# NVlabs/GLAMR

Measured on AMD Instinct MI355X. Metric: sequences/sec (300-frame, 1-person) end-to-end global_recon, higher is better.
Workload: dtype f32 (optimiser, init_data) / fp16x2-split MFMA with f32 accumulation (priors, LBS: every f32 operand as hi + lo fp16 planes, hi*hi + hi*lo + lo*hi)

## Files before the change

glamr_amd/csrc/nets.hip:

```cpp
#include "common.hpp"
#include "nn_kernels.hpp"
#include "nn_free.hpp"
#include "block_rt.hpp"
#include "rotmath.hpp"
#include <vector>
#include <cmath>
#include <cstring>
#include <map>
#include <mutex>

using namespace glamr;
using namespace glamr::nn;

namespace {

constexpr int D = 256, FF = 512, NZ = 128, WIN = 50, PAST = 10, CUR = 30, XLD = 96;

struct Lin { float* W = nullptr; float* b = nullptr; int N = 0, K = 0; unsigned short* Ws = nullptr;
             double rowabs = 0, babs = 0, wabs = 0; };
struct LN { float* g = nullptr; float* b = nullptr; double bound = 0; };
struct EncLayer { Lin qkv, o, f1, f2; LN n1, n2; };
struct DecLayer { Lin sa_qkv, sa_o, ca_q, ca_kv, ca_o, f1, f2; LN n1, n2, n3; };

struct HostT {
// ... 299 lines not shown
  __syncthreads();
  rt.scan(xy, n, 2, false);
  rt.scan(xy + 1, n, 2, false);
  for (int t = threadIdx.x; t < max_len; t += blockDim.x) {
    float tr[3] = {0.f, 0.f, 0.f}, aa[3] = {0.f, 0.f, 0.f};
    if (t < n) {
      const float base[4] = {0.5f, 0.5f, 0.5f, 0.5f};
      float hq[4], R[9], lq[4], q1[4], q[4];
      rm::heading_quat(theta[t], hq);
      rm::rot6d_to_rotmat(L + t * 11 + 3, R);
      rm::rotmat_to_quat(R, lq);
      rm::quat_mul(hq, lq, q1);
      rm::quat_mul(q1, base, q);
      rm::quat_to_aa(q, aa);
      tr[0] = xy[t * 2]; tr[1] = xy[t * 2 + 1]; tr[2] = L[t * 11 + 2];
    }
    for (int c = 0; c < 3; ++c) { trans[((size_t)b * max_len + t) * 3 + c] = tr[c]; orient[((size_t)b * max_len + t) * 3 + c] = aa[c]; }
  }
}

struct Ws {
  float *pose, *x, *h0, *h1, *qkv, *att, *tmp, *ff, *ctxkv, *qbuf, *pz, *z, *zproj, *dq, *y;
  float *tx, *tg, *th, *tq, *tmean, *trow, *traw, *tscr;
  float *gx, *q2, *qpz;
  float *te, *tcat, *e6, *tqz, *tloc;
  unsigned char* mask; int* lens; int* lens2;
  size_t total; int Tpad;
};
Ws ws_layout(int B, int max_len, char* base) {
  Ws w{};
  int nwin = (max_len - PAST + CUR - 1) / CUR;
  if (nwin < 1) nwin = 1;
  w.Tpad = std::max(max_len, (nwin - 1) * CUR + WIN);
  size_t off = 0;
  auto take = [&](size_t nfloats) { float* p = reinterpret_cast<float*>(base + off); off = align_up(off + (nfloats + 32 * 1024) * sizeof(float), 256); return p; };
  const size_t MW = (size_t)B * WIN, MT = (size_t)B * max_len;
  w.pose = take((size_t)B * w.Tpad * XLD);
  w.x = take(MW * XLD); w.h0 = take(MW * D); w.h1 = take(MW * D); w.qkv = take(MW * 3 * D); w.att = take(MW * D); w.tmp = take(MW * D);
  w.ff = take(MW * FF); w.ctxkv = take(MW * 2 * D); w.qbuf = take(MW * D); w.pz = take((size_t)B * 2 * D); w.z = take((size_t)B * NZ);
  w.zproj = take((size_t)B * FF); w.dq = take(MW * D); w.y = take(MW * 128);
  w.tx = take(MT * XLD); w.tg = take(MT * 1024); w.th = take(MT * D); w.tq = take(MT * D); w.tmean = take((size_t)B * D); w.trow = take((size_t)B * FF);
  w.traw = take(MT * 64); w.tscr = take(MT * 3);
  w.gx = take(MW * XLD); w.q2 = take((size_t)B * 2 * D); w.qpz = take((size_t)B * 2 * D);
  w.te = take(MT * D); w.tcat = take(MT * FF); w.e6 = take(MT * 32); w.tqz = take((size_t)B * D); w.tloc = take(MT * 11);
  w.mask = reinterpret_cast<unsigned char*>(take((MW + 3) / 4 + 64));
  w.lens = reinterpret_cast<int*>(take((size_t)B + 64));
  w.lens2 = reinterpret_cast<int*>(take((size_t)B + 64));
  w.total = off;
  return w;
}

#define RC(expr) do { int _rc = (expr); if (_rc) return _rc; } while (0)

thread_local int tl_fp32 = 0;
thread_local int tl_free = 0;
inline size_t cp(int col) { return tl_free ? (size_t)col * 32 : (size_t)col; }
inline bool free_wanted(int flags) {
  const char* e = std::getenv("GLAMR_NETS_FREE");
  return e ? std::atoi(e) != 0 : (flags & GLAMR_NETS_COSCHEDULE) != 0;
}

__global__ __launch_bounds__(64) void attention_f32_kernel(const float* Q, int ldq, const float* K, const float* V, int ldk, const unsigned char* key_mask,
                                                           float* O, int ldo, int Lq, int Lk, int q_shared) {
  __shared__ float sK[64][33], sV[64][33];
  __shared__ unsigned char sM[64];
  const int b = blockIdx.x, h = blockIdx.y, lane = threadIdx.x;
  for (int idx = lane; idx < 64 * 32; idx += 64) {
    const int j = idx >> 5, d = idx & 31;
    sK[j][d] = j < Lk ? K[(size_t)(b * Lk + j) * ldk + h * 32 + d] : 0.f;
    sV[j][d] = j < Lk ? V[(size_t)(b * Lk + j) * ldk + h * 32 + d] : 0.f;
  }
  sM[lane] = (lane < Lk) ? (key_mask ? key_mask[(size_t)b * Lk + lane] : 0) : 1;
  __syncthreads();
  if (lane >= Lq) return;
  float q[32], sc[64], o[32];
  for (int d = 0; d < 32; ++d) { q[d] = Q[(size_t)((q_shared ? 0 : b * Lq) + lane) * ldq + h * 32 + d]; o[d] = 0.f; }
  float mx = -3.0e38f;
  for (int j = 0; j < Lk; ++j) {
    float s = 0.f;
    for (int d = 0; d < 32; ++d) s = fmaf(q[d], sK[j][d], s);
    sc[j] = s * 0.17677669529663687f;
    if (!sM[j]) mx = fmaxf(mx, sc[j]);
  }
  float sum = 0.f;
  for (int j = 0; j < Lk; ++j) { const float e = sM[j] ? 0.f : expf(sc[j] - mx); sc[j] = e; sum += e; }
  const float inv = sum > 0.f ? 1.0f / sum : 0.f;
  for (int j = 0; j < Lk; ++j) { const float p = sc[j] * inv; for (int d = 0; d < 32; ++d) o[d] = fmaf(p, sV[j][d], o[d]); }
  for (int d = 0; d < 32; ++d) O[(size_t)(b * Lq + lane) * ldo + h * 32 + d] = o[d];
}

template <class... A>
void launch_attention(dim3 grid, dim3 block, size_t lds, hipStream_t st, const float* Q, int ldq, const float* K, const float* V, int ldk,
                      const unsigned char* mask, float* O, int ldo, int Lq, int Lk, int q_shared) {
  if (tl_fp32) hipLaunchKernelGGL(attention_f32_kernel, grid, dim3(64), 0, st, Q, ldq, K, V, ldk, mask, O, ldo, Lq, Lk, q_shared);
  else if (tl_free) hipLaunchKernelGGL(attention_free_kernel, dim3(grid.x * 8), dim3(64), 0, st, Q, ldq, K, V, ldk, mask, O, ldo, Lq, Lk, q_shared);
  else hipLaunchKernelGGL(attention_mfma_kernel, grid, block, lds, st, Q, ldq, K, V, ldk, mask, O, ldo, Lq, Lk, q_shared);
}

int ln(hipStream_t st, const float* X, const float* R, const LN& n, float* Y, int rows) {
  if (tl_free) { hipLaunchKernelGGL(ln_free_kernel, dim3((rows + 31) / 32), dim3(64), 0, st, X, R, n.g, n.b, Y, rows); return GLAMR_OK; }
  hipLaunchKernelGGL(add_layernorm_kernel, dim3((rows + 3) / 4), dim3(256), 0, st, X, R, n.g, n.b, Y, rows, D);
  return GLAMR_OK;
}
static const int FUSE_MIN_ROWS = [] { const char* e = std::getenv("GLAMR_NETS_FUSE_MIN_ROWS"); return e ? std::atoi(e) : 2048; }();
inline bool fuse_attention(int M) {
  static const bool no_fuse = std::getenv("GLAMR_NETS_NO_FUSE_ATTN") != nullptr || std::getenv("GLAMR_NETS_NO_FUSE") != nullptr;
  return !no_fuse && !tl_fp32 && !tl_free && M >= FUSE_MIN_ROWS;
}
int proj_ln(hipStream_t st, const Lin& L, const LN& n, const float* X, const float* R, float* Y, float* tmp, int M);
int mlp2(hipStream_t st, const Lin& L1, const Lin& L2, const LN* n, const float* X, int ldx, const float* R, float* Y, float* hidden, float* tmp, int M,
         int act2, int xl = -1);

inline bool small_rows_split(const Lin& L, int M, int ldx, int ldy, int ldr, int ldrb, bool bwd) {
  static const bool keep_fp32 = std::getenv("GLAMR_GEMM_SMALL_FP32") != nullptr || std::getenv("GLAMR_GEMM_FP32_MFMA") != nullptr;
  static const bool fwd_too = std::getenv("GLAMR_GEMM_SMALL_SPLIT_FWD") != nullptr;
  if (!bwd && !fwd_too) return false;
  return !keep_fp32 && !tl_fp32 && L.Ws && M > 0 && M < 2048 && L.K % 32 == 0 && ldx % 4 == 0 && ldy % 4 == 0 && ldr % 4 == 0 && ldrb % 4 == 0;
}

int lin(hipStream_t st, const Lin& L, const float* X, int ldx, float* Y, int ldy, int M, int act = ACT_NONE, const float* R = nullptr, int ldr = 0,
        const float* rowbias = nullptr, int rpg = 1, int ldrb = 0, int xl = -1, int yl = -1, bool bwd = false) {
  if (tl_free && L.Ws && M > 0) {
    if (L.K % 32 != 0 || ldx % 4 != 0 || ldy % 4 != 0) return fail(GLAMR_E_INVALID, "gemm: K=%d must be a multiple of 32, ldx=%d / ldy=%d of 4", L.K, ldx, ldy);
    GemmArgs a{X, L.W, L.b, rowbias, R, Y, M, L.N, L.K, ldx, ldy, ldr, rpg, ldrb, act};
    a.Ws = L.Ws;
    a.ws_plane = (size_t)((L.N + 63) / 64 * 64) * L.K;
    a.x_frag = xl != 0;
    a.y_frag = yl != 0;
    return launch_gemm_free(st, a);
  }
  if (small_rows_split(L, M, ldx, ldy, R ? ldr : 4, rowbias ? ldrb : 4, bwd)) {
    GemmArgs a{X, L.W, L.b, rowbias, R, Y, M, L.N, L.K, ldx, ldy, ldr, rpg, ldrb, act};
    a.Ws = L.Ws;
    a.ws_plane = (size_t)((L.N + 63) / 64 * 64) * L.K;
    return launch_gemm_free(st, a);
  }
  return launch_gemm(st, X, ldx, L.W, L.b, Y, ldy, M, L.N, L.K, act, R, ldr, rowbias, rpg, ldrb, L.Ws);
}

int proj_ln(hipStream_t st, const Lin& L, const LN& n, const float* X, const float* R, float* Y, float* tmp, int M) {
  static const bool no_fuse = std::getenv("GLAMR_NETS_NO_FUSE") != nullptr;
  if (!no_fuse && !tl_free && M >= FUSE_MIN_ROWS && L.N == D && L.K == D && L.Ws)
    return launch_rows(st, X, D, M, D, nullptr, 0, nullptr, nullptr, 1, 0, L.Ws, (size_t)D * L.K, L.K, L.b, ACT_NONE, R, D, n.g, n.b, Y, D);
  static const bool res_in_ln = std::getenv("GLAMR_NETS_RES_IN_LN") != nullptr;
  if (tl_free && !res_in_ln) {
    RC(lin(st, L, X, D, tmp, D, M, ACT_NONE, R, D));
    return ln(st, tmp, nullptr, n, Y, M);
  }
  RC(lin(st, L, X, D, tmp, D, M));
  return ln(st, tmp, R, n, Y, M);
}
int mlp2(hipStream_t st, const Lin& L1, const Lin& L2, const LN* n, const float* X, int ldx, const float* R, float* Y, float* hidden, float* tmp, int M,
         int act2, int xl) {
  static const bool no_fuse = std::getenv("GLAMR_NETS_NO_FUSE") != nullptr;
  if (!no_fuse && !tl_free && M >= FUSE_MIN_ROWS && L1.N == FF && L2.N == D && L2.K == FF && L1.K <= D && L1.Ws && L2.Ws)
    return launch_rows(st, X, ldx, M, L1.K, L1.Ws, (size_t)FF * L1.K, L1.b, nullptr, 1, 0, L2.Ws, (size_t)D * L2.K, L2.K, L2.b, act2, R, D,
                       n ? n->g : nullptr, n ? n->b : nullptr, Y, D);
  RC(lin(st, L1, X, ldx, hidden, FF, M, ACT_RELU, nullptr, 0, nullptr, 1, 0, xl));
  if (!n) return lin(st, L2, hidden, FF, Y, D, M, act2, R, D);
  static const bool res_in_ln2 = std::getenv("GLAMR_NETS_RES_IN_LN") != nullptr;
  if (tl_free && !res_in_ln2) {
    RC(lin(st, L2, hidden, FF, tmp, D, M, act2, R, D));
    return ln(st, tmp, nullptr, *n, Y, M);
  }
  RC(lin(st, L2, hidden, FF, tmp, D, M, act2));
  return ln(st, tmp, R, *n, Y, M);
}

}


extern "C" int glamr_nets_create(glamr_nets** out, const float* ib, const glamr_tensor_desc* idesc, int n_inf, const float* tb,
                                 const glamr_tensor_desc* tdesc, int n_trj, const float* fk_rest_joints, const int32_t* parents) {
  GLAMR_REQUIRE(out && ib && idesc && tb && tdesc && fk_rest_joints && parents, "null argument");
  GLAMR_REQUIRE(n_inf == 144 && n_trj == 66, "expected the 144 / 66 tensors of the reference checkpoints (got %d / %d)", n_inf, n_trj);
  GLAMR_REQUIRE(idesc[0].rows == 256 && idesc[0].cols == 69 && idesc[118].rows == 69 && tdesc[58].rows == 11 && tdesc[4].rows == 512,
                "tensor table is not in checkpoint (state_dict) order");
  glamr_nets* h = new (std::nothrow) glamr_nets();
  if (!h) return fail(GLAMR_E_NOMEM, "out of host memory");
  Blob I{ib, idesc, n_inf}, Tj{tb, tdesc, n_trj};
  tl_allocs = &h->allocs;
  auto lin_plain = [&](Lin& L, const Blob& B, int iw) { const std::vector<double> bias = vec_of(B.get(iw + 1)); return up_lin(L, B.get(iw), &bias); };
  auto lnorm = [&](LN& n, const Blob& B, int i) {
    const std::vector<double> g = vec_of(B.get(i)), be = vec_of(B.get(i + 1));
    n.bound = 0;
    for (size_t k = 0; k < g.size(); ++k) n.bound = std::max(n.bound, std::fabs(g[k]) * std::sqrt(255.0) + std::fabs(be[k]));
// ... 236 lines not shown
    h->capture_lens = nullptr;
  }
  for (void* p : h->allocs) (void)hipFree(p);
  delete h;
  return GLAMR_OK;
}

extern "C" size_t glamr_nets_workspace_bytes(const glamr_nets* h, int n_seq, int max_len) {
  if (!h || n_seq <= 0 || max_len <= 0) return 0;
  return ws_layout(n_seq, max_len, nullptr).total;
}

namespace {

int encoder_layer(hipStream_t st, const EncLayer& E, Ws& w, float* h_in, float* h_out, int B) {
  const int M = B * WIN;
  if (fuse_attention(M)) {
    const size_t pl = (size_t)3 * D * D;
    RC(launch_qkv_attention(st, B, QkvAttnArgs{h_in, WIN, h_in, WIN, E.qkv.Ws, pl, E.qkv.b, 0, E.qkv.Ws, pl, E.qkv.b, 8, 16, w.mask, w.att, D}));
  } else {
    RC(lin(st, E.qkv, h_in, D, w.qkv, 3 * D, M));
    launch_attention( dim3(B, 8), dim3(64), 0, st, w.qkv, 3 * D, w.qkv + cp(D), w.qkv + cp(2 * D), 3 * D, w.mask, w.att, D, WIN, WIN, 0);
  }
  RC(proj_ln(st, E.o, E.n1, w.att, h_in, h_out, w.tmp, M));
  RC(mlp2(st, E.f1, E.f2, &E.n2, h_out, D, h_out, h_out, w.ff, w.tmp, M, ACT_NONE));
  return GLAMR_OK;
}

int decoder_layer(hipStream_t st, const DecLayer& Dl, Ws& w, float* x, const float* ctx, int B, int Lq) {
  const int M = B * Lq;
  if (fuse_attention(M)) {
    const size_t pl = (size_t)3 * D * D;
    RC(launch_qkv_attention(st, B, QkvAttnArgs{x, Lq, x, Lq, Dl.sa_qkv.Ws, pl, Dl.sa_qkv.b, 0, Dl.sa_qkv.Ws, pl, Dl.sa_qkv.b, 8, 16, nullptr, w.att, D}));
  } else {
    RC(lin(st, Dl.sa_qkv, x, D, w.qkv, 3 * D, M));
    launch_attention( dim3(B, 8), dim3(64), 0, st, w.qkv, 3 * D, w.qkv + cp(D), w.qkv + cp(2 * D), 3 * D, (const unsigned char*)nullptr, w.att, D, Lq, Lq, 0);
  }
  RC(proj_ln(st, Dl.sa_o, Dl.n1, w.att, x, x, w.tmp, M));
  if (fuse_attention(M)) {
    RC(launch_qkv_attention(st, B, QkvAttnArgs{x, Lq, ctx, WIN, Dl.ca_q.Ws, (size_t)D * D, Dl.ca_q.b, 0, Dl.ca_kv.Ws, (size_t)2 * D * D, Dl.ca_kv.b, 0, 8, w.mask,
                                               w.att, D}));
  } else {
    RC(lin(st, Dl.ca_q, x, D, w.qbuf, D, M));
    RC(lin(st, Dl.ca_kv, ctx, D, w.ctxkv, 2 * D, B * WIN));
    launch_attention( dim3(B, 8), dim3(64), 0, st, w.qbuf, D, w.ctxkv, w.ctxkv + cp(D), 2 * D, w.mask, w.att, D, Lq, WIN, 0);
  }
  RC(proj_ln(st, Dl.ca_o, Dl.n2, w.att, x, x, w.tmp, M));
  RC(mlp2(st, Dl.f1, Dl.f2, &Dl.n3, x, D, x, x, w.ff, w.tmp, M, ACT_NONE));
  return GLAMR_OK;
}

}

namespace {


__global__ void window_in_kernel(const float* in_pose, const float* frame_mask, float* x, unsigned char* mask) {
  const int b = blockIdx.x, j = blockIdx.y, c = threadIdx.x;
  x[((size_t)b * WIN + j) * XLD + c] = c < 69 ? in_pose[((size_t)b * WIN + j) * 69 + c] : 0.0f;
  if (c == 0 && mask) mask[(size_t)b * WIN + j] = frame_mask[(size_t)b * WIN + j] == 1.0f ? 0 : 1;
}
__global__ void posterior_rows_kernel(const float* gx, float* x32) {
  const int b = blockIdx.x, r = blockIdx.y, c = threadIdx.x;
  x32[((size_t)b * 32 + r) * XLD + c] = r < 2 ? 0.0f : gx[((size_t)b * WIN + PAST + r - 2) * XLD + c];
}
__global__ void take_rows_kernel(const float* src, int rows_per_seq, int n_take, float* dst) {
  const int b = blockIdx.x, i = blockIdx.y, k = threadIdx.x;
  dst[((size_t)b * n_take + i) * D + k] = src[((size_t)b * rows_per_seq + i) * D + k];
}
__global__ void dist_out_kernel(const float* pz, float* out) {
  const int b = blockIdx.x, k = threadIdx.x;
// ... 128 lines not shown
    if (q_out) hipLaunchKernelGGL(dist_out_kernel, dim3(B), dim3(NZ), 0, st, w.qpz, q_out);
  }
  RC(lin(st, h->prior_kv, ctx, D, w.ctxkv, 2 * D, M));
  launch_attention( dim3(B, 8), dim3(64), 0, st, h->prior_q, D, w.ctxkv, w.ctxkv + cp(D), 2 * D, w.mask, w.att, D, 2, WIN, 1);
  RC(lin(st, h->prior_o, w.att, D, w.tmp, D, B * 2));
  hipLaunchKernelGGL(tile_rows_kernel, dim3((B * 2 * D + 255) / 256), dim3(64), 0, st, w.dq, h->prior_x1, 2, B * 2 * D, tl_free);
  RC(ln(st, w.tmp, w.dq, h->prior_n2, w.dq, B * 2));
  RC(lin(st, h->prior_f1, w.dq, D, w.ff, FF, B * 2, ACT_RELU));
  RC(lin(st, h->prior_f2, w.ff, FF, w.tmp, D, B * 2));
  RC(ln(st, w.tmp, w.dq, h->prior_n3, w.dq, B * 2));
  RC(lin(st, h->prior_pz, w.dq, D, w.pz, D, B * 2, ACT_NONE, nullptr, 0, nullptr, 1, 0, -1, 0));
  if (p_out) hipLaunchKernelGGL(dist_out_kernel, dim3(B), dim3(NZ), 0, st, w.pz, p_out);
  if (mode == GLAMR_VAE_INFER) hipLaunchKernelGGL(reparam_infiller_kernel, dim3(B), dim3(64), 0, st, w.pz, eps, eps_stride, w.z, B);
  else if (mode == GLAMR_VAE_TRAIN) hipLaunchKernelGGL(reparam_infiller_kernel, dim3(B), dim3(64), 0, st, w.qpz, eps, eps_stride, w.z, B);
  else hipLaunchKernelGGL(mode_infiller_kernel, dim3(B), dim3(NZ), 0, st, w.qpz, w.z);
  RC(lin(st, h->dec_z, w.z, NZ, w.zproj, D, B, ACT_NONE, nullptr, 0, nullptr, 1, 0, 0, 0));
  hipLaunchKernelGGL(build_queries_kernel, dim3(B, CUR), dim3(64), 0, st, w.zproj, h->dec_pe, w.dq, tl_free);
  RC(decoder_layer(st, h->dec[0], w, w.dq, ctx, B, CUR));
  RC(decoder_layer(st, h->dec[1], w, w.dq, ctx, B, CUR));
  RC(mlp2(st, h->out1, h->out2, nullptr, w.dq, D, nullptr, w.tmp, w.ff, w.tmp, B * CUR, ACT_RELU));
  RC(lin(st, h->outfc, w.tmp, D, w.y, 128, B * CUR, ACT_NONE, nullptr, 0, nullptr, 1, 0, -1, 0));
  return GLAMR_OK;
}

#include "nets_tape.hpp"

void bilstm(glamr_nets* h, hipStream_t st, const float* G, float* const hh[2], const int* lens, float* H, int max_len, int B) {
  LstmArgs la{G, hh[0], hh[1], lens, H, max_len};
  if (B >= 512 && !tl_fp32) hipLaunchKernelGGL(lstm_mfma_kernel, dim3((B + 15) / 16, 2), dim3(512), 0, st, la, B);
  else hipLaunchKernelGGL(lstm_kernel, dim3(B, 2), dim3(512), 0, st, la);
}

int traj_pass(glamr_nets* h, hipStream_t st, Ws& w, int B, int max_len, const int* lens_run, int mode, const float* eps, float* q_out, float* p_out,
              const float* init, int ldinit, float* out_orig, float* out_local, float* out_trans, float* out_orient, float* out_orient_q) {
  const int MT = B * max_len;
  RC(mlp2(st, h->t_in1, h->t_in2, nullptr, w.tx, XLD, nullptr, w.th, w.tg, w.tq, MT, ACT_RELU, 0));
  for (int l = 0; l < 2; ++l) {
    RC(lin(st, h->t_ih[l], w.th, D, w.tg, 1024, MT, ACT_NONE, nullptr, 0, nullptr, 1, 0, l == 0 ? -1 : 0, 0));
    tl_free = 0;
    bilstm(h, st, w.tg, h->t_hh[l], lens_run, w.th, max_len, B);
  }
  RC(mlp2(st, h->t_out1, h->t_out2, nullptr, w.th, D, nullptr, w.th, w.tg, w.tq, MT, ACT_RELU, 0));
  if (mode != GLAMR_VAE_INFER) {
    RC(lin(st, h->te_in1, w.e6, 32, w.tg, FF, MT, ACT_RELU));
    RC(lin(st, h->te_in2, w.tg, FF, w.te, D, MT, ACT_RELU));
    for (int l = 0; l < 2; ++l) {
      RC(lin(st, h->te_ih[l], w.te, D, w.tg, 1024, MT));
// ... 57 lines not shown
  hipLaunchKernelGGL(fk_joints_kernel, dim3(B, (max_len + FK_FRAMES - 1) / FK_FRAMES), dim3(256), 0, st, w.pose, w.Tpad, max_len, w.lens, h->rest_joints, h->parents, w.tx);
  return traj_pass(h, st, w, B, max_len, w.lens, GLAMR_VAE_INFER, traj_eps, nullptr, nullptr, nullptr, 0, nullptr, out_local_traj, out_trans, out_orient, nullptr);
}
}

extern "C" int glamr_nets_infer(glamr_nets* h, int B, int max_len, const int32_t* lens_host, const float* body_pose, const float* visible,
                                const float* motion_eps, int n_win_max, const float* traj_eps, float* out_pose, float* out_local_traj,
                                float* out_trans, float* out_orient, int flags, void* workspace, void* stream_) {
  const bool do_infill = flags & GLAMR_NETS_INFILL, do_traj = flags & GLAMR_NETS_TRAJ;
  GLAMR_REQUIRE(h && lens_host && body_pose && workspace && (do_infill || do_traj), "null argument / empty flags");
  GLAMR_REQUIRE(!do_infill || (visible && motion_eps && out_pose), "infilling needs visible, motion_eps and out_pose");
  GLAMR_REQUIRE(!do_traj || (traj_eps && out_local_traj && out_trans && out_orient), "trajectory prediction needs traj_eps and its three outputs");
  GLAMR_REQUIRE(B > 0 && max_len > PAST, "need n_seq > 0 and max_len > %d", PAST);
  int longest = 0;
  for (int b = 0; b < B; ++b) {
    GLAMR_REQUIRE(lens_host[b] > PAST && lens_host[b] <= max_len, "sequence %d has length %d (need %d < len <= max_len)", b, lens_host[b], PAST);
    longest = std::max(longest, (int)lens_host[b]);
  }
  const int n_win = (longest - PAST + CUR - 1) / CUR;
  GLAMR_REQUIRE(!do_infill || n_win <= n_win_max, "motion_eps holds %d windows per sequence, %d needed", n_win_max, n_win);
  hipStream_t st = static_cast<hipStream_t>(stream_);
  tl_fp32 = h->fp32_only ? 1 : 0;
  tl_free = (!tl_fp32 && free_wanted(flags) && (size_t)B * WIN >= (size_t)FUSE_MIN_ROWS) ? 1 : 0;
  Ws w = ws_layout(B, max_len, static_cast<char*>(workspace));
  hipStreamCaptureStatus cap = hipStreamCaptureStatusNone;
  const bool outer_capture = st != nullptr && hipStreamIsCapturing(st, &cap) == hipSuccess && cap == hipStreamCaptureStatusActive;
  const int32_t* lens_src = lens_host;
  if (outer_capture) {
    std::lock_guard<std::mutex> lock(h->graph_mu);
    GLAMR_REQUIRE(h->capture_lens && h->capture_lens_used + (size_t)B <= CAPTURE_LENS_INTS,
                  "the handle's table for calls recorded into caller graphs is full (%zu lengths); destroy and re-create the handle", CAPTURE_LENS_INTS);
    int32_t* pinned = h->capture_lens + h->capture_lens_used;
    h->capture_lens_used += (size_t)B;
    std::memcpy(pinned, lens_host, (size_t)B * sizeof(int32_t));
    lens_src = pinned;
  }
  static const bool lens_memcpy = std::getenv("GLAMR_NETS_LENS_MEMCPY") != nullptr;
  if (outer_capture && !lens_memcpy) hipLaunchKernelGGL(copy_ints_kernel, dim3((B + 255) / 256), dim3(256), 0, st, w.lens, lens_src, B);
  else GLAMR_HIP_CHECK(hipMemcpyAsync(w.lens, lens_src, (size_t)B * sizeof(int), hipMemcpyHostToDevice, st));
  auto enqueue = [&]() -> int {
    return enqueue_infer(h, st, w, B, max_len, n_win, n_win_max, do_infill, do_traj, body_pose, visible, motion_eps, traj_eps, out_pose, out_local_traj, out_trans,
                         out_orient);
  };
  static const bool no_graph = std::getenv("GLAMR_NETS_NO_GRAPH") != nullptr;
  if (!no_graph && !outer_capture) {
    glamr_nets::GraphKey key;
    std::memset(&key, 0, sizeof(key));
    key.v[0] = B; key.v[1] = max_len; key.v[2] = n_win; key.v[3] = flags | (tl_free << 16); key.v[4] = n_win_max;
    const void* ptrs[9] = {body_pose, visible, motion_eps, traj_eps, out_pose, out_local_traj, out_trans, out_orient, workspace};
    for (int i = 0; i < 9; ++i) key.p[i] = ptrs[i];
    std::lock_guard<std::mutex> lock(h->graph_mu);
    auto it = h->graphs.find(key);
    if (it == h->graphs.end()) {
      if (h->graphs.size() >= GRAPH_CACHE_MAX) {
        auto old = h->graphs.begin();
        for (auto jt = h->graphs.begin(); jt != h->graphs.end(); ++jt) if (jt->second.last_use < old->second.last_use) old = jt;
        if (old->second.exec) {
          (void)hipDeviceSynchronize();
          (void)hipGraphExecDestroy(old->second.exec);
        }
        h->graphs.erase(old);
      }
      it = h->graphs.emplace(key, glamr_nets::GraphEntry()).first;
    }
    {
      glamr_nets::GraphEntry& e = it->second;
      e.last_use = ++h->graph_clock;
      if (e.exec) {
        GLAMR_HIP_CHECK(hipGraphLaunch(e.exec, st));
        return GLAMR_OK;
      }
// ... 191 lines not shown
```

glamr_amd/csrc/nn_free.hpp:

```cpp
#pragma once
#include <type_traits>
#include "nn_kernels.hpp"

namespace glamr {
namespace nn {

__host__ __device__ inline size_t x32_off(int row, int col, int ld) {
  return (((size_t)(row >> 5) * (ld >> 4) + (col >> 4)) * 64 + (row & 31) + 32 * ((col >> 3) & 1)) * 8 + (col & 7);
}

__device__ __forceinline__ float lane_xor32(float x) {
  const unsigned u = __float_as_uint(x);
  const auto r = __builtin_amdgcn_permlane32_swap(u, u, false, false);
  return __uint_as_float((threadIdx.x & 32) ? r[0] : r[1]);
}

template <int KS, int C, int PD, int MAXW>
__global__ __launch_bounds__(64, MAXW) void gemm_free_kernel(GemmArgs a) {
  const int lane = threadIdx.x, c = lane & 31, kg = lane >> 5;
  const int ncb = (a.N + 32 * C - 1) / (32 * C);
  const int lin = blockIdx.x, grp = lin / (8 * ncb), within = lin % (8 * ncb);
  const int rb = grp * 8 + (within & 7), cb = within >> 3;
  if (rb * 32 >= a.M) return;
  const int m0 = rb * 32, n0 = cb * 32 * C;
  const int ksteps = KS ? KS : a.K / 16;
  const int row = m0 + c;
  const float* xp = a.x_frag ? a.X + ((size_t)rb * (a.ldx >> 4) * 64 + lane) * 8 : a.X + (size_t)min(row, a.M - 1) * a.ldx + 8 * kg;
  const int xstep = a.x_frag ? 512 : 16;
  const int ntile = (a.N + 63) / 64 * 2;
  const uint4* wp[2][C];
#pragma unroll
  for (int p = 0; p < 2; ++p)
#pragma unroll
    for (int j = 0; j < C; ++j) wp[p][j] = reinterpret_cast<const uint4*>(a.Ws + p * a.ws_plane) + ((size_t)min(cb * C + j, ntile - 1) * ksteps) * 64 + lane;
  f32x16 acc[C];
#pragma unroll
  for (int j = 0; j < C; ++j) acc[j] = (f32x16){0};
  f32x4 xr[PD + 1][2];
  uint4 wr[PD + 1][2][C];
  auto fetch = [&](int ks, int slot) {
    xr[slot][0] = *reinterpret_cast<const f32x4*>(xp + (size_t)ks * xstep);
    xr[slot][1] = *reinterpret_cast<const f32x4*>(xp + (size_t)ks * xstep + 4);
#pragma unroll
    for (int p = 0; p < 2; ++p)
#pragma unroll
      for (int j = 0; j < C; ++j) wr[slot][p][j] = wp[p][j][(size_t)ks * 64];
  };
  auto step = [&](int slot) {
    const float x[8] = {xr[slot][0][0], xr[slot][0][1], xr[slot][0][2], xr[slot][0][3], xr[slot][1][0], xr[slot][1][1], xr[slot][1][2], xr[slot][1][3]};
    f16x8 xh, xl;
#ifdef GLAMR_GEMM_NOSPLIT
    xh = __builtin_bit_cast(f16x8, xr[slot][0]); xl = __builtin_bit_cast(f16x8, xr[slot][1]);
#else
    split8(x, xh, xl);
#endif
#pragma unroll
    for (int j = 0; j < C; ++j) acc[j] = __builtin_amdgcn_mfma_f32_32x32x16_f16(__builtin_bit_cast(f16x8, wr[slot][1][j]), xh, acc[j], 0, 0, 0);
#pragma unroll
    for (int j = 0; j < C; ++j) acc[j] = __builtin_amdgcn_mfma_f32_32x32x16_f16(__builtin_bit_cast(f16x8, wr[slot][0][j]), xl, acc[j], 0, 0, 0);
#pragma unroll
    for (int j = 0; j < C; ++j) acc[j] = __builtin_amdgcn_mfma_f32_32x32x16_f16(__builtin_bit_cast(f16x8, wr[slot][0][j]), xh, acc[j], 0, 0, 0);
  };
  if constexpr (KS > 0) {
#pragma unroll
    for (int d = 0; d < PD; ++d) if (d < KS) fetch(d, d);
#pragma unroll
    for (int ks = 0; ks < KS; ++ks) {
      if (ks + PD < KS) fetch(ks + PD, (ks + PD) % (PD + 1));
      __builtin_amdgcn_sched_barrier(0);
      step(ks % (PD + 1));
      __builtin_amdgcn_sched_barrier(0);
    }
  } else {
    for (int d = 0; d < PD; ++d) if (d < ksteps) fetch(d, d);
    for (int k3 = 0; k3 < ksteps; k3 += PD + 1) {
#pragma unroll
      for (int u = 0; u <= PD; ++u) {
        const int ks = k3 + u;
        if (ks >= ksteps) break;
        if (ks + PD < ksteps) fetch(ks + PD, (u + PD) % (PD + 1));
        __builtin_amdgcn_sched_barrier(0);
        step(u);
        __builtin_amdgcn_sched_barrier(0);
      }
    }
  }
  if (row >= a.M) return;
  const int rbrow = a.rowbias ? (a.rows_per_group > 0 ? row / a.rows_per_group : row % (-a.rows_per_group)) : 0;
  if (n0 + 32 * C <= a.N || a.y_frag) {
    auto emit = [&](auto has_b, auto has_rb, auto relu, auto has_r, auto frag) {
#pragma unroll
      for (int j = 0; j < C; ++j)
#pragma unroll
        for (int i = 0; i < 4; ++i) {
          const int n = n0 + 32 * j + 8 * i + 4 * kg;
          if (n >= a.N) continue;
          f32x4 v = {acc[j][4 * i], acc[j][4 * i + 1], acc[j][4 * i + 2], acc[j][4 * i + 3]};
          if (decltype(has_b)::value) v += *reinterpret_cast<const f32x4*>(a.bias + n);
          if (decltype(has_rb)::value) v += *reinterpret_cast<const f32x4*>(a.rowbias + (size_t)rbrow * a.ldrb + n);
          if (decltype(relu)::value) { v[0] = fmaxf(v[0], 0.f); v[1] = fmaxf(v[1], 0.f); v[2] = fmaxf(v[2], 0.f); v[3] = fmaxf(v[3], 0.f); }
          if (decltype(has_r)::value) v += *reinterpret_cast<const f32x4*>(a.R + (decltype(frag)::value ? x32_off(row, n, a.ldr) : (size_t)row * a.ldr + n));
          *reinterpret_cast<f32x4*>(a.Y + (decltype(frag)::value ? x32_off(row, n, a.ldy) : (size_t)row * a.ldy + n)) = v;
        }
    };
    using T = std::true_type; using F = std::false_type;
    auto pick_frag = [&](auto has_b, auto has_rb, auto relu, auto has_r) { if (a.y_frag) emit(has_b, has_rb, relu, has_r, T{}); else emit(has_b, has_rb, relu, has_r, F{}); };
    auto pick_r = [&](auto has_b, auto has_rb, auto relu) { if (a.R) pick_frag(has_b, has_rb, relu, T{}); else pick_frag(has_b, has_rb, relu, F{}); };
    auto pick_relu = [&](auto has_b, auto has_rb) { if (a.act == ACT_RELU) pick_r(has_b, has_rb, T{}); else pick_r(has_b, has_rb, F{}); };
    auto pick_rb = [&](auto has_b) { if (a.rowbias) pick_relu(has_b, T{}); else pick_relu(has_b, F{}); };
    if (a.bias) pick_rb(T{}); else pick_rb(F{});
// ... 21 lines not shown
          if (a.act == ACT_RELU) s = fmaxf(s, 0.f);
          if (a.R) s += a.R[(size_t)row * a.ldr + n + e];
          a.Y[(size_t)row * a.ldy + n + e] = s;
        }
      }
    }
}

template <int C, int PD, int MAXW>
inline int launch_gemm_free_t(hipStream_t st, const GemmArgs& a) {
  const int ncb = (a.N + 32 * C - 1) / (32 * C), nrb = (a.M + 31) / 32;
  const dim3 grid((unsigned)((nrb + 7) / 8 * 8 * ncb)), block(64);
  switch (a.K / 16) {
    case 2: hipLaunchKernelGGL((gemm_free_kernel<2, C, PD, MAXW>), grid, block, 0, st, a); break;
    case 6: hipLaunchKernelGGL((gemm_free_kernel<6, C, PD, MAXW>), grid, block, 0, st, a); break;
    case 8: hipLaunchKernelGGL((gemm_free_kernel<8, C, PD, MAXW>), grid, block, 0, st, a); break;
    case 16: hipLaunchKernelGGL((gemm_free_kernel<16, C, PD, MAXW>), grid, block, 0, st, a); break;
    case 32: hipLaunchKernelGGL((gemm_free_kernel<32, C, PD, MAXW>), grid, block, 0, st, a); break;
    case 48: hipLaunchKernelGGL((gemm_free_kernel<48, C, PD, MAXW>), grid, block, 0, st, a); break;
    default: hipLaunchKernelGGL((gemm_free_kernel<0, C, PD, MAXW>), grid, block, 0, st, a); break;
  }
  return GLAMR_OK;
}
inline int launch_gemm_free(hipStream_t st, const GemmArgs& a) {
  if ((a.x_frag && a.ldx % 16 != 0) || (a.y_frag && (a.ldy % 16 != 0 || (a.R && a.ldr % 16 != 0) || a.ldy < (a.N + 3) / 4 * 4)))
    return fail(GLAMR_E_INVALID, "fragment-major GEMM: ldx=%d / ldy=%d / ldr=%d must be multiples of 16", a.ldx, a.ldy, a.ldr);
#ifndef GLAMR_FREE_GEMM_CFG
#define GLAMR_FREE_GEMM_CFG 2, 1, 4
#endif
  if (a.M <= 128 && !a.x_frag && !a.y_frag) return launch_gemm_free_t<1, 1, 4>(st, a);
  return launch_gemm_free_t<GLAMR_FREE_GEMM_CFG>(st, a);
}

__global__ __launch_bounds__(64, 4) void ln_free_kernel(const float* X, const float* R, const float* gamma, const float* beta, float* Y, int rows) {
  const int lane = threadIdx.x, kg = lane >> 5;
  const size_t base = ((size_t)blockIdx.x * 16 * 64 + lane) * 8;
  auto load = [&](int s, f32x4& u, f32x4& w) {
    u = *reinterpret_cast<const f32x4*>(X + base + (size_t)s * 512);
    w = *reinterpret_cast<const f32x4*>(X + base + (size_t)s * 512 + 4);
    if (R) { u += *reinterpret_cast<const f32x4*>(R + base + (size_t)s * 512); w += *reinterpret_cast<const f32x4*>(R + base + (size_t)s * 512 + 4); }
  };
  float sum = 0.f;
#pragma unroll 4
  for (int s = 0; s < 16; ++s) {
    f32x4 u, w;
    load(s, u, w);
    sum += ((u[0] + u[1]) + (u[2] + u[3])) + ((w[0] + w[1]) + (w[2] + w[3]));
  }
  sum += lane_xor32(sum);
  const float mean = sum * (1.0f / 256.0f);
  float sq = 0.f;
#pragma unroll 4
  for (int s = 0; s < 16; ++s) {
    f32x4 u, w;
    load(s, u, w);
    u -= mean; w -= mean;
    sq += ((u[0] * u[0] + u[1] * u[1]) + (u[2] * u[2] + u[3] * u[3])) + ((w[0] * w[0] + w[1] * w[1]) + (w[2] * w[2] + w[3] * w[3]));
  }
  sq += lane_xor32(sq);
  const float rstd = 1.0f / sqrtf(sq * (1.0f / 256.0f) + 1e-5f);
  if ((int)blockIdx.x * 32 + (lane & 31) >= rows) return;
#pragma unroll 4
  for (int s = 0; s < 16; ++s) {
    f32x4 u, w;
    load(s, u, w);
    const int col = 16 * s + 8 * kg;
    u = (u - mean) * rstd * *reinterpret_cast<const f32x4*>(gamma + col) + *reinterpret_cast<const f32x4*>(beta + col);
    w = (w - mean) * rstd * *reinterpret_cast<const f32x4*>(gamma + col + 4) + *reinterpret_cast<const f32x4*>(beta + col + 4);
    *reinterpret_cast<f32x4*>(Y + base + (size_t)s * 512) = u;
    *reinterpret_cast<f32x4*>(Y + base + (size_t)s * 512 + 4) = w;
  }
}

__global__ __launch_bounds__(64, 4) void attention_free_kernel(const float* Q, int ldq, const float* K, const float* V, int ldk, const unsigned char* key_mask,
                                                               float* O, int ldo, int Lq, int Lk, int q_shared) {
  const int b = blockIdx.x >> 3, h = blockIdx.x & 7, lane = threadIdx.x, c = lane & 31, kg = lane >> 5;
  const unsigned char mk = (lane < Lk) ? (key_mask ? key_mask[(size_t)b * Lk + lane] : 0) : 1;
  const unsigned long long masked = __ballot(mk != 0);
  const bool two_k = Lk > 32, two_q = Lq > 32;
  auto row_frag = [&](const float* base, int ld, int grow, bool frag, bool valid, int s, float scale, f16x8& hi, f16x8& lo) {
    float x[8];
    if (valid) {
      const float* p = base + (frag ? x32_off(grow, h * 32 + 16 * s + 8 * kg, ld) : (size_t)grow * ld + h * 32 + 16 * s + 8 * kg);
      const f32x4 u = *reinterpret_cast<const f32x4*>(p), w = *reinterpret_cast<const f32x4*>(p + 4);
#pragma unroll
// ... 99 lines not shown
```

glamr_amd/csrc/nn_kernels.hpp:

```cpp
#pragma once
#include <cstdlib>
#include <cstdio>
#include <type_traits>
#include "common.hpp"

namespace glamr {
namespace nn {

typedef float f32x16 __attribute__((ext_vector_type(16)));
typedef float f32x4 __attribute__((ext_vector_type(4)));

constexpr int GT_M = 64, GT_N = 64, GT_K = 32, GT_LD = 36;

enum Act { ACT_NONE = 0, ACT_RELU = 1 };

struct GemmArgs {
  const float* X; const float* W; const float* bias; const float* rowbias; const float* R; float* Y;
  int M, N, K, ldx, ldy, ldr, rows_per_group, ldrb, act;
  const unsigned short* Ws = nullptr;
  size_t ws_plane = 0;
  int x_frag = 0, y_frag = 0;
};

__global__ __launch_bounds__(256) void gemm_kernel(GemmArgs a) {
  __shared__ __attribute__((aligned(16))) float sA[2][GT_M * GT_LD];
  __shared__ __attribute__((aligned(16))) float sB[2][GT_N * GT_LD];
  const int tid = threadIdx.x, lane = tid & 63, wave = tid >> 6;
  const int wm = wave >> 1, wn = wave & 1;
  const int col = lane & 31, half = lane >> 5;
  const int m0 = blockIdx.y * GT_M, n0 = blockIdx.x * GT_N;
  f32x16 acc = {0};
  const int r0 = tid >> 3, c4 = (tid & 7) * 4;
  constexpr int GT_PF = 4;
  const int nchunks = a.K / GT_K;
  f32x4 va[GT_PF][2], vb[GT_PF][2];
  const float* xa[2];
  const float* xb[2];
#pragma unroll
  for (int q = 0; q < 2; ++q) {
    const int r = r0 + q * 32;
    xa[q] = a.X + (size_t)min(m0 + r, a.M - 1) * a.ldx + c4;
    xb[q] = a.W + (size_t)(n0 + r) * a.K + c4;
  }
  auto fetch = [&](int c, int slot) {
// ... 1042 lines not shown
```

Measured before the change: 30230.

## Fuse LayerNorm row sums into GEMM epilogue and pre-split FFN hidden to fp16

Adds two GEMM epilogue modes to the free-path kernel. One writes per-row partial sums after the residual add, so the following LayerNorm skips its first pass over the row. The other has the first FFN linear emit fp16 hi/lo planes directly, so the second linear reads them without re-splitting. This cuts LayerNorm memory traffic and split ALU work, at the cost of an extra sums buffer, more template instantiations, and fp16 hidden storage that is the same size as f32. LN loop unroll is also raised.

```diff
diff --git a/glamr_amd/csrc/nets.hip b/glamr_amd/csrc/nets.hip
--- a/glamr_amd/csrc/nets.hip
+++ b/glamr_amd/csrc/nets.hip
@@ -345,6 +345,7 @@
 struct Ws {
   float *pose, *x, *h0, *h1, *qkv, *att, *tmp, *ff, *ctxkv, *qbuf, *pz, *z, *zproj, *dq, *y;
   float *tx, *tg, *th, *tq, *tmean, *trow, *traw, *tscr;
+  float* lsum;
   float *gx, *q2, *qpz;
   float *te, *tcat, *e6, *tqz, *tloc;
   unsigned char* mask; int* lens; int* lens2;
@@ -364,6 +365,7 @@
   w.zproj = take((size_t)B * FF); w.dq = take(MW * D); w.y = take(MW * 128);
   w.tx = take(MT * XLD); w.tg = take(MT * 1024); w.th = take(MT * D); w.tq = take(MT * D); w.tmean = take((size_t)B * D); w.trow = take((size_t)B * FF);
   w.traw = take(MT * 64); w.tscr = take(MT * 3);
+  w.lsum = take(MW * LN_SUMS_LD);
   w.gx = take(MW * XLD); w.q2 = take((size_t)B * 2 * D); w.qpz = take((size_t)B * 2 * D);
   w.te = take(MT * D); w.tcat = take(MT * FF); w.e6 = take(MT * 32); w.tqz = take((size_t)B * D); w.tloc = take(MT * 11);
   w.mask = reinterpret_cast<unsigned char*>(take((MW + 3) / 4 + 64));
@@ -377,6 +379,7 @@
 
 thread_local int tl_fp32 = 0;
 thread_local int tl_free = 0;
+thread_local int tl_lnsums = 0, tl_presplit = 0;
 inline size_t cp(int col) { return tl_free ? (size_t)col * 32 : (size_t)col; }
 inline bool free_wanted(int flags) {
   const char* e = std::getenv("GLAMR_NETS_FREE");
@@ -420,8 +423,8 @@
   else hipLaunchKernelGGL(attention_mfma_kernel, grid, block, lds, st, Q, ldq, K, V, ldk, mask, O, ldo, Lq, Lk, q_shared);
 }
 
-int ln(hipStream_t st, const float* X, const float* R, const LN& n, float* Y, int rows) {
-  if (tl_free) { hipLaunchKernelGGL(ln_free_kernel, dim3((rows + 31) / 32), dim3(64), 0, st, X, R, n.g, n.b, Y, rows); return GLAMR_OK; }
+int ln(hipStream_t st, const float* X, const float* R, const LN& n, float* Y, int rows, const float* sums = nullptr) {
+  if (tl_free) { hipLaunchKernelGGL(ln_free_kernel, dim3((rows + 31) / 32), dim3(64), 0, st, X, R, n.g, n.b, Y, rows, sums); return GLAMR_OK; }
   hipLaunchKernelGGL(add_layernorm_kernel, dim3((rows + 3) / 4), dim3(256), 0, st, X, R, n.g, n.b, Y, rows, D);
   return GLAMR_OK;
 }
@@ -430,9 +433,9 @@
   static const bool no_fuse = std::getenv("GLAMR_NETS_NO_FUSE_ATTN") != nullptr || std::getenv("GLAMR_NETS_NO_FUSE") != nullptr;
   return !no_fuse && !tl_fp32 && !tl_free && M >= FUSE_MIN_ROWS;
 }
-int proj_ln(hipStream_t st, const Lin& L, const LN& n, const float* X, const float* R, float* Y, float* tmp, int M);
+int proj_ln(hipStream_t st, const Lin& L, const LN& n, const float* X, const float* R, float* Y, float* tmp, int M, float* sums = nullptr);
 int mlp2(hipStream_t st, const Lin& L1, const Lin& L2, const LN* n, const float* X, int ldx, const float* R, float* Y, float* hidden, float* tmp, int M,
-         int act2, int xl = -1);
+         int act2, int xl = -1, float* sums = nullptr);
 
 inline bool small_rows_split(const Lin& L, int M, int ldx, int ldy, int ldr, int ldrb, bool bwd) {
   static const bool keep_fp32 = std::getenv("GLAMR_GEMM_SMALL_FP32") != nullptr || std::getenv("GLAMR_GEMM_FP32_MFMA") != nullptr;
@@ -442,7 +445,8 @@
 }
 
 int lin(hipStream_t st, const Lin& L, const float* X, int ldx, float* Y, int ldy, int M, int act = ACT_NONE, const float* R = nullptr, int ldr = 0,
-        const float* rowbias = nullptr, int rpg = 1, int ldrb = 0, int xl = -1, int yl = -1, bool bwd = false) {
+        const float* rowbias = nullptr, int rpg = 1, int ldrb = 0, int xl = -1, int yl = -1, bool bwd = false, int x16 = 0, int y16 = 0,
+        float* ysums = nullptr) {
   if (tl_free && L.Ws && M > 0) {
     if (L.K % 32 != 0 || ldx % 4 != 0 || ldy % 4 != 0) return fail(GLAMR_E_INVALID, "gemm: K=%d must be a multiple of 32, ldx=%d / ldy=%d of 4", L.K, ldx, ldy);
     GemmArgs a{X, L.W, L.b, rowbias, R, Y, M, L.N, L.K, ldx, ldy, ldr, rpg, ldrb, act};
@@ -450,6 +454,9 @@
     a.ws_plane = (size_t)((L.N + 63) / 64 * 64) * L.K;
     a.x_frag = xl != 0;
     a.y_frag = yl != 0;
+    a.x16 = x16;
+    a.y16 = y16;
+    a.y_sums = ysums;
     return launch_gemm_free(st, a);
   }
   if (small_rows_split(L, M, ldx, ldy, R ? ldr : 4, rowbias ? ldrb : 4, bwd)) {
@@ -461,30 +468,33 @@
   return launch_gemm(st, X, ldx, L.W, L.b, Y, ldy, M, L.N, L.K, act, R, ldr, rowbias, rpg, ldrb, L.Ws);
 }
 
-int proj_ln(hipStream_t st, const Lin& L, const LN& n, const float* X, const float* R, float* Y, float* tmp, int M) {
+int proj_ln(hipStream_t st, const Lin& L, const LN& n, const float* X, const float* R, float* Y, float* tmp, int M, float* sums) {
   static const bool no_fuse = std::getenv("GLAMR_NETS_NO_FUSE") != nullptr;
   if (!no_fuse && !tl_free && M >= FUSE_MIN_ROWS && L.N == D && L.K == D && L.Ws)
     return launch_rows(st, X, D, M, D, nullptr, 0, nullptr, nullptr, 1, 0, L.Ws, (size_t)D * L.K, L.K, L.b, ACT_NONE, R, D, n.g, n.b, Y, D);
   static const bool res_in_ln = std::getenv("GLAMR_NETS_RES_IN_LN") != nullptr;
   if (tl_free && !res_in_ln) {
-    RC(lin(st, L, X, D, tmp, D, M, ACT_NONE, R, D));
-    return ln(st, tmp, nullptr, n, Y, M);
+    float* ys = tl_lnsums && sums && R && L.N == D ? sums : nullptr;
+    RC(lin(st, L, X, D, tmp, D, M, ACT_NONE, R, D, nullptr, 1, 0, -1, -1, false, 0, 0, ys));
+    return ln(st, tmp, nullptr, n, Y, M, ys);
   }
   RC(lin(st, L, X, D, tmp, D, M));
   return ln(st, tmp, R, n, Y, M);
 }
 int mlp2(hipStream_t st, const Lin& L1, const Lin& L2, const LN* n, const float* X, int ldx, const float* R, float* Y, float* hidden, float* tmp, int M,
-         int act2, int xl) {
+         int act2, int xl, float* sums) {
   static const bool no_fuse = std::getenv("GLAMR_NETS_NO_FUSE") != nullptr;
   if (!no_fuse && !tl_free && M >= FUSE_MIN_ROWS && L1.N == FF && L2.N == D && L2.K == FF && L1.K <= D && L1.Ws && L2.Ws)
     return launch_rows(st, X, ldx, M, L1.K, L1.Ws, (size_t)FF * L1.K, L1.b, nullptr, 1, 0, L2.Ws, (size_t)D * L2.K, L2.K, L2.b, act2, R, D,
                        n ? n->g : nullptr, n ? n->b : nullptr, Y, D);
-  RC(lin(st, L1, X, ldx, hidden, FF, M, ACT_RELU, nullptr, 0, nullptr, 1, 0, xl));
-  if (!n) return lin(st, L2, hidden, FF, Y, D, M, act2, R, D);
+  const int ps = tl_free && tl_presplit && xl != 0 && L1.N == FF && L2.K == FF;
+  RC(lin(st, L1, X, ldx, hidden, FF, M, ACT_RELU, nullptr, 0, nullptr, 1, 0, xl, -1, false, 0, ps));
+  if (!n) return lin(st, L2, hidden, FF, Y, D, M, act2, R, D, nullptr, 1, 0, -1, -1, false, ps);
   static const bool res_in_ln2 = std::getenv("GLAMR_NETS_RES_IN_LN") != nullptr;
   if (tl_free && !res_in_ln2) {
-    RC(lin(st, L2, hidden, FF, tmp, D, M, act2, R, D));
-    return ln(st, tmp, nullptr, *n, Y, M);
+    float* ys = tl_lnsums && sums && R && act2 == ACT_NONE && L2.N == D ? sums : nullptr;
+    RC(lin(st, L2, hidden, FF, tmp, D, M, act2, R, D, nullptr, 1, 0, -1, -1, false, ps, 0, ys));
+    return ln(st, tmp, nullptr, *n, Y, M, ys);
   }
   RC(lin(st, L2, hidden, FF, tmp, D, M, act2));
   return ln(st, tmp, R, *n, Y, M);
@@ -767,8 +777,8 @@
     RC(lin(st, E.qkv, h_in, D, w.qkv, 3 * D, M));
     launch_attention( dim3(B, 8), dim3(64), 0, st, w.qkv, 3 * D, w.qkv + cp(D), w.qkv + cp(2 * D), 3 * D, w.mask, w.att, D, WIN, WIN, 0);
   }
-  RC(proj_ln(st, E.o, E.n1, w.att, h_in, h_out, w.tmp, M));
-  RC(mlp2(st, E.f1, E.f2, &E.n2, h_out, D, h_out, h_out, w.ff, w.tmp, M, ACT_NONE));
+  RC(proj_ln(st, E.o, E.n1, w.att, h_in, h_out, w.tmp, M, w.lsum));
+  RC(mlp2(st, E.f1, E.f2, &E.n2, h_out, D, h_out, h_out, w.ff, w.tmp, M, ACT_NONE, -1, w.lsum));
   return GLAMR_OK;
 }
 
@@ -781,7 +791,7 @@
     RC(lin(st, Dl.sa_qkv, x, D, w.qkv, 3 * D, M));
     launch_attention( dim3(B, 8), dim3(64), 0, st, w.qkv, 3 * D, w.qkv + cp(D), w.qkv + cp(2 * D), 3 * D, (const unsigned char*)nullptr, w.att, D, Lq, Lq, 0);
   }
-  RC(proj_ln(st, Dl.sa_o, Dl.n1, w.att, x, x, w.tmp, M));
+  RC(proj_ln(st, Dl.sa_o, Dl.n1, w.att, x, x, w.tmp, M, w.lsum));
   if (fuse_attention(M)) {
     RC(launch_qkv_attention(st, B, QkvAttnArgs{x, Lq, ctx, WIN, Dl.ca_q.Ws, (size_t)D * D, Dl.ca_q.b, 0, Dl.ca_kv.Ws, (size_t)2 * D * D, Dl.ca_kv.b, 0, 8, w.mask,
                                                w.att, D}));
@@ -790,8 +800,8 @@
     RC(lin(st, Dl.ca_kv, ctx, D, w.ctxkv, 2 * D, B * WIN));
     launch_attention( dim3(B, 8), dim3(64), 0, st, w.qbuf, D, w.ctxkv, w.ctxkv + cp(D), 2 * D, w.mask, w.att, D, Lq, WIN, 0);
   }
-  RC(proj_ln(st, Dl.ca_o, Dl.n2, w.att, x, x, w.tmp, M));
-  RC(mlp2(st, Dl.f1, Dl.f2, &Dl.n3, x, D, x, x, w.ff, w.tmp, M, ACT_NONE));
+  RC(proj_ln(st, Dl.ca_o, Dl.n2, w.att, x, x, w.tmp, M, w.lsum));
+  RC(mlp2(st, Dl.f1, Dl.f2, &Dl.n3, x, D, x, x, w.ff, w.tmp, M, ACT_NONE, -1, w.lsum));
   return GLAMR_OK;
 }
 
@@ -966,7 +976,6 @@
   RC(lin(st, h->outfc, w.tmp, D, w.y, 128, B * CUR, ACT_NONE, nullptr, 0, nullptr, 1, 0, -1, 0));
   return GLAMR_OK;
 }
-
 #include "nets_tape.hpp"
 
 void bilstm(glamr_nets* h, hipStream_t st, const float* G, float* const hh[2], const int* lens, float* H, int max_len, int B) {
@@ -1070,6 +1079,8 @@
   hipStream_t st = static_cast<hipStream_t>(stream_);
   tl_fp32 = h->fp32_only ? 1 : 0;
   tl_free = (!tl_fp32 && free_wanted(flags) && (size_t)B * WIN >= (size_t)FUSE_MIN_ROWS) ? 1 : 0;
+  tl_lnsums = tl_free && std::getenv("GLAMR_NETS_NO_LN_SUMS") == nullptr;
+  tl_presplit = tl_free && std::getenv("GLAMR_NETS_NO_PRESPLIT") == nullptr;
   Ws w = ws_layout(B, max_len, static_cast<char*>(workspace));
   hipStreamCaptureStatus cap = hipStreamCaptureStatusNone;
   const bool outer_capture = st != nullptr && hipStreamIsCapturing(st, &cap) == hipSuccess && cap == hipStreamCaptureStatusActive;
@@ -1094,7 +1105,7 @@
   if (!no_graph && !outer_capture) {
     glamr_nets::GraphKey key;
     std::memset(&key, 0, sizeof(key));
-    key.v[0] = B; key.v[1] = max_len; key.v[2] = n_win; key.v[3] = flags | (tl_free << 16); key.v[4] = n_win_max;
+    key.v[0] = B; key.v[1] = max_len; key.v[2] = n_win; key.v[3] = flags | (tl_free << 16) | (tl_lnsums << 17) | (tl_presplit << 18); key.v[4] = n_win_max;
     const void* ptrs[9] = {body_pose, visible, motion_eps, traj_eps, out_pose, out_local_traj, out_trans, out_orient, workspace};
     for (int i = 0; i < 9; ++i) key.p[i] = ptrs[i];
     std::lock_guard<std::mutex> lock(h->graph_mu);
diff --git a/glamr_amd/csrc/nn_free.hpp b/glamr_amd/csrc/nn_free.hpp
--- a/glamr_amd/csrc/nn_free.hpp
+++ b/glamr_amd/csrc/nn_free.hpp
@@ -5,9 +5,18 @@
 namespace glamr {
 namespace nn {
 
+typedef _Float16 f16x4 __attribute__((ext_vector_type(4)));
+
 __host__ __device__ inline size_t x32_off(int row, int col, int ld) {
   return (((size_t)(row >> 5) * (ld >> 4) + (col >> 4)) * 64 + (row & 31) + 32 * ((col >> 3) & 1)) * 8 + (col & 7);
 }
+__host__ __device__ inline size_t x16_off(int row, int col, int ld) {
+  return (((size_t)(row >> 5) * (ld >> 4) + (col >> 4)) * 128 + (row & 31) + 32 * ((col >> 3) & 1)) * 8 + (col & 7);
+}
+
+constexpr int LN_SUMS_LD = 32;
+enum { X_F32 = 0, X_16 = 2 };
+enum { E_PLAIN = 0, E_SUMS = 1, E_SPLIT = 2 };
 
 __device__ __forceinline__ float lane_xor32(float x) {
   const unsigned u = __float_as_uint(x);
@@ -15,7 +24,7 @@
   return __uint_as_float((threadIdx.x & 32) ? r[0] : r[1]);
 }
 
-template <int KS, int C, int PD, int MAXW>
+template <int KS, int C, int PD, int MAXW, int XM = X_F32, int EM = E_PLAIN>
 __global__ __launch_bounds__(64, MAXW) void gemm_free_kernel(GemmArgs a) {
   const int lane = threadIdx.x, c = lane & 31, kg = lane >> 5;
   const int ncb = (a.N + 32 * C - 1) / (32 * C);
@@ -25,7 +34,8 @@
   const int m0 = rb * 32, n0 = cb * 32 * C;
   const int ksteps = KS ? KS : a.K / 16;
   const int row = m0 + c;
-  const float* xp = a.x_frag ? a.X + ((size_t)rb * (a.ldx >> 4) * 64 + lane) * 8 : a.X + (size_t)min(row, a.M - 1) * a.ldx + 8 * kg;
+  const float* xp = XM == X_16 ? a.X + (size_t)rb * (a.ldx >> 4) * 512 + lane * 4
+                  : a.x_frag ? a.X + ((size_t)rb * (a.ldx >> 4) * 64 + lane) * 8 : a.X + (size_t)min(row, a.M - 1) * a.ldx + 8 * kg;
   const int xstep = a.x_frag ? 512 : 16;
   const int ntile = (a.N + 63) / 64 * 2;
   const uint4* wp[2][C];
@@ -40,7 +50,7 @@
   uint4 wr[PD + 1][2][C];
   auto fetch = [&](int ks, int slot) {
     xr[slot][0] = *reinterpret_cast<const f32x4*>(xp + (size_t)ks * xstep);
-    xr[slot][1] = *reinterpret_cast<const f32x4*>(xp + (size_t)ks * xstep + 4);
+    xr[slot][1] = *reinterpret_cast<const f32x4*>(xp + (size_t)ks * xstep + (XM == X_16 ? 256 : 4));
 #pragma unroll
     for (int p = 0; p < 2; ++p)
 #pragma unroll
@@ -52,7 +62,8 @@
 #ifdef GLAMR_GEMM_NOSPLIT
     xh = __builtin_bit_cast(f16x8, xr[slot][0]); xl = __builtin_bit_cast(f16x8, xr[slot][1]);
 #else
-    split8(x, xh, xl);
+    if constexpr (XM == X_16) { xh = __builtin_bit_cast(f16x8, xr[slot][0]); xl = __builtin_bit_cast(f16x8, xr[slot][1]); }
+    else split8(x, xh, xl);
 #endif
 #pragma unroll
     for (int j = 0; j < C; ++j) acc[j] = __builtin_amdgcn_mfma_f32_32x32x16_f16(__builtin_bit_cast(f16x8, wr[slot][1][j]), xh, acc[j], 0, 0, 0);
@@ -86,6 +97,47 @@
     }
   }
   if (row >= a.M) return;
+  using T = std::true_type; using F = std::false_type;
+  if constexpr (EM == E_SUMS) {
+    f32x4 sums = {0.f, 0.f, 0.f, 0.f};
+#pragma unroll
+    for (int j = 0; j < C; ++j)
+#pragma unroll
+      for (int i = 0; i < 4; ++i) {
+        const int n = n0 + 32 * j + 8 * i + 4 * kg;
+        f32x4 v = {acc[j][4 * i], acc[j][4 * i + 1], acc[j][4 * i + 2], acc[j][4 * i + 3]};
+        v += *reinterpret_cast<const f32x4*>(a.bias + n);
+        v += *reinterpret_cast<const f32x4*>(a.R + x32_off(row, n, a.ldr));
+        *reinterpret_cast<f32x4*>(a.Y + x32_off(row, n, a.ldy)) = v;
+        const float mine = (v[0] + v[1]) + (v[2] + v[3]), other = lane_xor32(mine);
+        const float s8 = kg ? other + mine : mine + other;
+        if ((i & 1) == kg) sums[2 * j + (i >> 1)] = s8;
+      }
+    *reinterpret_cast<f32x4*>(a.y_sums + (size_t)row * LN_SUMS_LD + 16 * kg + (n0 >> 4)) = sums;
+    return;
+  }
+  if constexpr (EM == E_SPLIT) {
+    _Float16* yh = reinterpret_cast<_Float16*>(a.Y);
+    auto emit = [&](auto relu) {
+#pragma unroll
+      for (int j = 0; j < C; ++j)
+#pragma unroll
+        for (int i = 0; i < 4; ++i) {
+          const int n = n0 + 32 * j + 8 * i + 4 * kg;
+          f32x4 v = {acc[j][4 * i], acc[j][4 * i + 1], acc[j][4 * i + 2], acc[j][4 * i + 3]};
+          v += *reinterpret_cast<const f32x4*>(a.bias + n);
+          if (decltype(relu)::value) { v[0] = fmaxf(v[0], 0.f); v[1] = fmaxf(v[1], 0.f); v[2] = fmaxf(v[2], 0.f); v[3] = fmaxf(v[3], 0.f); }
+          f16x4 hi, lo;
+#pragma unroll
+          for (int e = 0; e < 4; ++e) { const _Float16 h = (_Float16)v[e]; hi[e] = h; lo[e] = (_Float16)(v[e] - (float)h); }
+          const size_t o = x16_off(row, n, a.ldy);
+          *reinterpret_cast<f16x4*>(yh + o) = hi;
+          *reinterpret_cast<f16x4*>(yh + o + 512) = lo;
+        }
+    };
+    if (a.act == ACT_RELU) emit(T{}); else emit(F{});
+    return;
+  }
   const int rbrow = a.rowbias ? (a.rows_per_group > 0 ? row / a.rows_per_group : row % (-a.rows_per_group)) : 0;
   if (n0 + 32 * C <= a.N || a.y_frag) {
     auto emit = [&](auto has_b, auto has_rb, auto relu, auto has_r, auto frag) {
@@ -153,17 +205,38 @@
   }
   return GLAMR_OK;
 }
+template <int C, int PD, int MAXW, int XM, int EM>
+inline int launch_gemm_free_m(hipStream_t st, const GemmArgs& a) {
+  const int ncb = (a.N + 32 * C - 1) / (32 * C), nrb = (a.M + 31) / 32;
+  const dim3 grid((unsigned)((nrb + 7) / 8 * 8 * ncb)), block(64);
+  if constexpr (XM == X_F32) if (a.K == 256) { hipLaunchKernelGGL((gemm_free_kernel<16, C, PD, MAXW, XM, EM>), grid, block, 0, st, a); return GLAMR_OK; }
+  if (a.K == 512) { hipLaunchKernelGGL((gemm_free_kernel<32, C, PD, MAXW, XM, EM>), grid, block, 0, st, a); return GLAMR_OK; }
+  return fail(GLAMR_E_INVALID, "gemm_free: K=%d in operand mode %d", a.K, XM);
+}
 inline int launch_gemm_free(hipStream_t st, const GemmArgs& a) {
   if ((a.x_frag && a.ldx % 16 != 0) || (a.y_frag && (a.ldy % 16 != 0 || (a.R && a.ldr % 16 != 0) || a.ldy < (a.N + 3) / 4 * 4)))
     return fail(GLAMR_E_INVALID, "fragment-major GEMM: ldx=%d / ldy=%d / ldr=%d must be multiples of 16", a.ldx, a.ldy, a.ldr);
 #ifndef GLAMR_FREE_GEMM_CFG
 #define GLAMR_FREE_GEMM_CFG 2, 1, 4
 #endif
+  const int xm = a.x16 ? X_16 : X_F32, em = a.y_sums ? E_SUMS : a.y16 ? E_SPLIT : E_PLAIN;
+  if (xm != X_F32 || em != E_PLAIN) {
+    constexpr int cfg[3] = {GLAMR_FREE_GEMM_CFG};
+    if ((xm != X_F32 && !a.x_frag) || (a.y_sums && a.y16) || (em != E_PLAIN && (!a.y_frag || !a.bias || a.rowbias || a.N % (32 * cfg[0]) != 0)) ||
+        (em == E_SUMS && (a.N != 256 || !a.R || a.act != ACT_NONE || cfg[0] != 2)) || (em == E_SPLIT && a.R))
+      return fail(GLAMR_E_INVALID, "gemm_free: unsupported operand / epilogue mode (M=%d N=%d K=%d modes %d / %d)", a.M, a.N, a.K, xm, em);
+    if (xm == X_16 && em == E_PLAIN) return launch_gemm_free_m<GLAMR_FREE_GEMM_CFG, X_16, E_PLAIN>(st, a);
+    if (xm == X_16 && em == E_SUMS) return launch_gemm_free_m<GLAMR_FREE_GEMM_CFG, X_16, E_SUMS>(st, a);
+    if (xm == X_F32 && em == E_SUMS) return launch_gemm_free_m<GLAMR_FREE_GEMM_CFG, X_F32, E_SUMS>(st, a);
+    if (xm == X_F32 && em == E_SPLIT) return launch_gemm_free_m<GLAMR_FREE_GEMM_CFG, X_F32, E_SPLIT>(st, a);
+    return fail(GLAMR_E_INVALID, "gemm_free: operand mode %d with epilogue %d is not built", xm, em);
+  }
   if (a.M <= 128 && !a.x_frag && !a.y_frag) return launch_gemm_free_t<1, 1, 4>(st, a);
   return launch_gemm_free_t<GLAMR_FREE_GEMM_CFG>(st, a);
 }
 
-__global__ __launch_bounds__(64, 4) void ln_free_kernel(const float* X, const float* R, const float* gamma, const float* beta, float* Y, int rows) {
+__global__ __launch_bounds__(64, 4) void ln_free_kernel(const float* X, const float* R, const float* gamma, const float* beta, float* Y, int rows,
+                                                        const float* sums) {
   const int lane = threadIdx.x, kg = lane >> 5;
   const size_t base = ((size_t)blockIdx.x * 16 * 64 + lane) * 8;
   auto load = [&](int s, f32x4& u, f32x4& w) {
@@ -172,16 +245,25 @@
     if (R) { u += *reinterpret_cast<const f32x4*>(R + base + (size_t)s * 512); w += *reinterpret_cast<const f32x4*>(R + base + (size_t)s * 512 + 4); }
   };
   float sum = 0.f;
-#pragma unroll 4
-  for (int s = 0; s < 16; ++s) {
-    f32x4 u, w;
-    load(s, u, w);
-    sum += ((u[0] + u[1]) + (u[2] + u[3])) + ((w[0] + w[1]) + (w[2] + w[3]));
+  if (sums) {
+    const f32x4* sp = reinterpret_cast<const f32x4*>(sums + ((size_t)blockIdx.x * 32 + (lane & 31)) * LN_SUMS_LD + 16 * kg);
+#pragma unroll
+    for (int v = 0; v < 4; ++v) {
+      const f32x4 q = sp[v];
+      sum += q[0]; sum += q[1]; sum += q[2]; sum += q[3];
+    }
+  } else {
+#pragma unroll 8
+    for (int s = 0; s < 16; ++s) {
+      f32x4 u, w;
+      load(s, u, w);
+      sum += ((u[0] + u[1]) + (u[2] + u[3])) + ((w[0] + w[1]) + (w[2] + w[3]));
+    }
   }
   sum += lane_xor32(sum);
   const float mean = sum * (1.0f / 256.0f);
   float sq = 0.f;
-#pragma unroll 4
+#pragma unroll 8
   for (int s = 0; s < 16; ++s) {
     f32x4 u, w;
     load(s, u, w);
@@ -191,7 +273,7 @@
   sq += lane_xor32(sq);
   const float rstd = 1.0f / sqrtf(sq * (1.0f / 256.0f) + 1e-5f);
   if ((int)blockIdx.x * 32 + (lane & 31) >= rows) return;
-#pragma unroll 4
+#pragma unroll 8
   for (int s = 0; s < 16; ++s) {
     f32x4 u, w;
     load(s, u, w);
diff --git a/glamr_amd/csrc/nn_kernels.hpp b/glamr_amd/csrc/nn_kernels.hpp
--- a/glamr_amd/csrc/nn_kernels.hpp
+++ b/glamr_amd/csrc/nn_kernels.hpp
@@ -20,6 +20,8 @@
   const unsigned short* Ws = nullptr;
   size_t ws_plane = 0;
   int x_frag = 0, y_frag = 0;
+  float* y_sums = nullptr;
+  int x16 = 0, y16 = 0;
 };
 
 __global__ __launch_bounds__(256) void gemm_kernel(GemmArgs a) {
```

Measured after the change: 30730 (median of 6 runs). 1.7% higher.
